# Chlumsky/msdfgen

Hardware: AMD Instinct MI355X
Metric: MSDF glyphs/sec (64x64, fp32) (higher is better)
Workload: dtype f64

## Files before the change

msdfgen_amd/csrc/msdf_ec_fast.hpp:

```cpp
#pragma once

#include "msdf_ec.hpp"

namespace msdfhip {

enum { EC_DEFER = 0x80 };

enum { EC_V_ERROR = 1,
       EC_V_CHECK = 2,
       EC_V_COND = 4,
       EC_V_HELD = 8 };
enum { EC_ORDER_EAGER = 0, EC_ORDER_LAZY = 1, EC_ORDER_LAZY_HELD = 2 };

MSDF_HD bool ecHasBasePass(const EcParams &p) { return p.distanceCheck == EC_DO_NOT_CHECK || (p.distanceCheck == EC_CHECK_AT_EDGE && p.mode != EC_MODE_EDGE_ONLY); }
MSDF_HD bool ecHasShapePass(const EcParams &p) { return p.distanceCheck == EC_ALWAYS_CHECK || p.distanceCheck == EC_CHECK_AT_EDGE; }
MSDF_HD bool ecLazyProtect(const EcParams &p) { return p.mode == EC_MODE_EDGE_PRIORITY && p.distanceCheck == EC_CHECK_AT_EDGE; }

struct FastCtx {
    double span;
    bool p1;
    bool pShape;
    bool basePass, shapePass;
    int order;
};

MSDF_HD int rangeTest2(const FastCtx &c, double at, double bt, double xt, float am, float bm, float xm) {
    const bool inversion = (am > .5f && bm > .5f && xm <= .5f) || (am < .5f && bm < .5f && xm >= .5f);
    const bool outside = medianf(am, bm, xm) != xm;
    const bool candBase = c.basePass && (inversion || (!c.p1 && outside));
    const bool candShape = c.shapePass && (inversion || (!c.pShape && outside));
    const bool candCond = c.order != EC_ORDER_EAGER && !inversion && outside;
    if (!(candBase || candShape || candCond))
        return 0;
    const double axSpan = (xt-at)*c.span, bxSpan = (bt-xt)*c.span;
    const int f = (xm >= am-axSpan && xm <= am+axSpan && xm >= bm-bxSpan && xm <= bm+bxSpan) ? 1 : 3;
    return (candBase ? f : 0)|(candShape ? f<<2 : 0)|(candCond && f == 3 ? 16 : 0);
}

MSDF_HD int judge(int flags) {
    const int cond = (flags&16) ? EC_V_COND : 0;
    if (flags&2)
        return EC_V_ERROR|cond;
    const int fs = (flags>>2)&3;
    if (fs&1)
        return ((fs&2) ? EC_V_ERROR : EC_V_CHECK)|cond;
    return cond;
}

MSDF_HD bool quadraticMayHaveRootInRange(double a, double b, double c) {
    if (a == 0 || fabs(b) > 1e12*fabs(a))
        return true;
    const double lo = .005, hi = .995;
    const double mag = fabs(a)+fabs(b)+fabs(c);
    const double eps = 1e-9*mag;
    const double flo = (a*lo+b)*lo+c, fhi = (a*hi+b)*hi+c;
    if (!(flo > eps && fhi > eps) && !(flo < -eps && fhi < -eps))
        return true;
    const double s = flo > 0 ? 1. : -1.;
    const double as = a*s, bs = b*s, cs = c*s;
    if (as <= 0)
        return false;
    if (!(-bs > 2*as*lo*(1-1e-9) && -bs < 2*as*hi*(1+1e-9)))
        return false;
    return !(4*as*cs-bs*bs > 1e-9*mag*mag);
}

MSDF_HD bool bernsteinMayHaveRoot(float dA, float dBC, float dD) {
    const float m = fmaxf(fmaxf(fabsf(dA), fabsf(dBC)), fabsf(dD));
    const float eps = 1e-5f*m;
    const float h = .5f*dBC;
    return !((dA > eps && h > eps && dD > eps) || (dA < -eps && h < -eps && dD < -eps));
}

MSDF_HD bool edgeBetweenTexelsChannelFast(const float *a, const float *b, int channel) {
    const double n = a[channel]-.5;
    const double d = a[channel]-b[channel];
    if (!((n > 0 && d > 0 && n < d) || (n < 0 && d < 0 && n > d)))
        return false;
    const double t = n/d;
    if (t > 0 && t < 1) {
        float c[3] = { mixf(a[0], b[0], t), mixf(a[1], b[1], t), mixf(a[2], b[2], t) };
        return medianf(c[0], c[1], c[2]) == c[channel];
    }
    return false;
}

MSDF_HD int edgeBetweenTexelsFast(const float *a, const float *b) {
    return 1*(int) edgeBetweenTexelsChannelFast(a, b, 0)+2*(int) edgeBetweenTexelsChannelFast(a, b, 1)+4*(int) edgeBetweenTexelsChannelFast(a, b, 2);
}

template <class Sink>
MSDF_HD int diagonalPairFast(const FastCtx &cx, float am, float dm, const float *a, const float *l, const float *q,
                             float dA, float dBC, float dD, float l0, float q0, float l1, float q1, Sink &sink) {
    const double qa = dD-dBC+dA, qb = dBC-dA-dA, qc = dA;
    if (!quadraticMayHaveRootInRange(qa, qb, qc))
        return 0;
    double t[2];
    const int solutions = solveQuadratic(t, qa, qb, qc);
    int verdict = 0;
    for (int i = 0; i < solutions; ++i) {
        if (t[i] > MSDF_ARTIFACT_T_EPSILON && t[i] < 1-MSDF_ARTIFACT_T_EPSILON) {
            const float xm = interpolatedMedianQuad(a, l, q, t[i]);
            int rangeFlags = rangeTest2(cx, 0, 1, t[i], am, dm, xm);
            const double tEx0 = -.5*l0/q0, tEx1 = -.5*l1/q1;
            if (tEx0 > 0 && tEx0 < 1) {
                double tEnd0 = 0, tEnd1 = 1;
                float em0 = am, em1 = dm;
                const float ex = interpolatedMedianQuad(a, l, q, tEx0);
                if (tEx0 > t[i])
                    tEnd1 = tEx0, em1 = ex;
                else
                    tEnd0 = tEx0, em0 = ex;
                rangeFlags |= rangeTest2(cx, tEnd0, tEnd1, t[i], em0, em1, xm);
            }
            if (tEx1 > 0 && tEx1 < 1) {
                double tEnd0 = 0, tEnd1 = 1;
                float em0 = am, em1 = dm;
                const float ex = interpolatedMedianQuad(a, l, q, tEx1);
                if (tEx1 > t[i])
                    tEnd1 = tEx1, em1 = ex;
                else
                    tEnd0 = tEx1, em0 = ex;
                rangeFlags |= rangeTest2(cx, tEnd0, tEnd1, t[i], em0, em1, xm);
            }
            const int v = judge(rangeFlags);
            verdict |= v;
            if (v&EC_V_CHECK) {
                const bool held = (verdict&EC_V_COND) != 0;
                if (held)
                    verdict |= EC_V_HELD;
                if (held == (cx.order == EC_ORDER_LAZY_HELD))
                    sink(t[i]);
            }
            if (verdict&EC_V_ERROR)
                return verdict;
        }
    }
    return verdict;
}

struct Neighbourhood {
    float v[3][3][3];
    float dev[3][3];
    unsigned valid;
};

MSDF_HD float ecTexelDeviation(const float *t) { return fabsf(medianf(t[0], t[1], t[2])-.5f); }

MSDF_HD void loadNeighbourhood(Neighbourhood &nb, const SdfView &sdf, int x, int yn) {
    nb.valid = 0;
    MSDF_UNROLL
    for (int dy = -1; dy <= 1; ++dy) {
        MSDF_UNROLL
        for (int dx = -1; dx <= 1; ++dx) {
            const int nx = x+dx, ny = yn+dy;
            const bool in = nx >= 0 && ny >= 0 && nx < sdf.w && ny < sdf.h;
            const float *t = sdf.native(in ? nx : x, in ? ny : yn);
            nb.v[dy+1][dx+1][0] = t[0], nb.v[dy+1][dx+1][1] = t[1], nb.v[dy+1][dx+1][2] = t[2];
            nb.dev[dy+1][dx+1] = ecTexelDeviation(t);
            if (in)
                nb.valid |= 1u<<((dy+1)*3+(dx+1));
        }
    }
}

template <class Emit>
MSDF_HD void texelProtectPairs(const Neighbourhood &nb, const EcParams &p, Emit &emit) {
    const float sdev = nb.dev[1][1];
    MSDF_UNROLL
    for (int dy = -1; dy <= 1; ++dy) {
        MSDF_UNROLL
        for (int dx = -1; dx <= 1; ++dx) {
            if (!dx && !dy)
                continue;
            if (!(nb.valid&(1u<<((dy+1)*3+(dx+1)))))
                continue;
            const float radius = dy == 0 ? p.radiusH : dx == 0 ? p.radiusV : p.radiusD;
            const float odev = nb.dev[dy+1][dx+1];
            const bool selfIsA = dy > 0 || (dy == 0 && dx > 0);
            const float sum = selfIsA ? sdev+odev : odev+sdev;
            if (sum < radius)
                emit((dy+1)*3+(dx+1));
        }
    }
}

MSDF_HD bool evaluateProtectPair(const float *self, const float *other, int m) {
    const int dy = m/3-1, dx = m%3-1;
    const bool selfIsA = dy > 0 || (dy == 0 && dx > 0);
    const int mask = selfIsA ? edgeBetweenTexelsFast(self, other) : edgeBetweenTexelsFast(other, self);
    return extremeChannelInMask(self, medianf(self[0], self[1], self[2]), mask);
}

MSDF_HD bool protectedByEdgesNb(const Neighbourhood &nb, const EcParams &p) {
    struct Items {
        unsigned char m[8];
        int n;
        MSDF_HD void operator()(int mm) { m[n++] = (unsigned char) mm; }
    } items;
    items.n = 0;
    texelProtectPairs(nb, p, items);
    for (int i = 0; i < items.n; ++i)
        if (evaluateProtectPair(nb.v[1][1], nb.v[items.m[i]/3][items.m[i]%3], items.m[i]))
            return true;
    return false;
}

MSDF_HD int ecNeighbourDx(int k) { return k < 4 ? (k == 0 ? -1 : k == 2 ? 1 : 0) : ((k&1) ? 1 : -1); }
MSDF_HD int ecNeighbourDy(int k) { return k < 4 ? (k == 1 ? -1 : k == 3 ? 1 : 0) : ((k&2) ? 1 : -1); }

template <class Emit>
MSDF_HD void texelCandidatePairs(const Neighbourhood &nb, Emit &emit) {
    const float *c = nb.v[1][1];
    const float cdev = nb.dev[1][1];
    MSDF_UNROLL
    for (int k = 0; k < 4; ++k) {
        const int dx = k == 0 ? -1 : k == 2 ? 1 : 0, dy = k == 1 ? -1 : k == 3 ? 1 : 0;
        if (!(nb.valid&(1u<<((dy+1)*3+(dx+1)))))
            continue;
        const float *b = nb.v[dy+1][dx+1];
        if (!(cdev >= nb.dev[dy+1][dx+1]))
            continue;
        MSDF_UNROLL
        for (int j = 0; j < 3; ++j) {
            const int i0 = j, i1 = j == 2 ? 0 : j+1;
            const float dA = c[i1]-c[i0], dB = b[i1]-b[i0];
            if ((dA > 0 && dB < 0) || (dA < 0 && dB > 0))
                emit(k, j);
        }
    }
    MSDF_UNROLL
    for (int k = 4; k < 8; ++k) {
        const int dx = (k&1) ? 1 : -1, dy = (k&2) ? 1 : -1;
        if (!(nb.valid&(1u<<((dy+1)*3+(dx+1)))))
            continue;
        const float *d = nb.v[dy+1][dx+1];
        if (!(cdev >= nb.dev[dy+1][dx+1]))
            continue;
        const float *b = nb.v[1][dx+1], *cc = nb.v[dy+1][1];
        MSDF_UNROLL
        for (int j = 0; j < 3; ++j) {
            const int i0 = j, i1 = j == 2 ? 0 : j+1;
            const float dA = c[i1]-c[i0], dBC = b[i1]-b[i0]+cc[i1]-cc[i0], dD = d[i1]-d[i0];
            if (dA == 0 && dBC == 0 && dD == 0)
                continue;
            if (bernsteinMayHaveRoot(dA, dBC, dD))
                emit(k, j);
        }
    }
}

MSDF_HD float pick3(const float *v, int i) { return i == 0 ? v[0] : i == 1 ? v[1] : v[2]; }

template <class Sink>
MSDF_HD int evaluatePair(const float *c, const float *n, const float *hb, const float *vc, const EcParams &p, bool p1, int flip, int k, int j, Sink &sink,
                         int order = EC_ORDER_EAGER) {
    FastCtx cx;
    cx.basePass = ecHasBasePass(p);
    cx.shapePass = ecHasShapePass(p);
    cx.order = order;
    cx.p1 = order != EC_ORDER_EAGER || p1;
    cx.pShape = (p.distanceCheck == EC_CHECK_AT_EDGE) ? true : cx.p1;
    const int dx = ecNeighbourDx(k), dy = ecNeighbourDy(k);
    const int i0 = j, i1 = j == 2 ? 0 : j+1;
    const float cm = medianf(c[0], c[1], c[2]), nm = medianf(n[0], n[1], n[2]);
    if (k < 4) {
        if (order == EC_ORDER_LAZY_HELD)
            return 0;
        cx.span = dy == 0 ? p.hSpan : p.vSpan;
        const float dA = pick3(c, i1)-pick3(c, i0), dB = pick3(n, i1)-pick3(n, i0);
        const double t = (double) dA/(dA-dB);
        if (t > MSDF_ARTIFACT_T_EPSILON && t < 1-MSDF_ARTIFACT_T_EPSILON) {
            const float xm = interpolatedMedianLin(c, n, t);
            const int v = judge(rangeTest2(cx, 0, 1, t, cm, nm, xm));
            if (v&EC_V_CHECK)
                sink(t, dx, flip ? -dy : dy);
            return v;
        }
        return 0;
    }
    cx.span = p.dSpan;
    const float *a = c, *b = hb, *cc = vc, *d = n;
    const float abc[3] = { a[0]-b[0]-cc[0], a[1]-b[1]-cc[1], a[2]-b[2]-cc[2] };
    const float l[3] = { -a[0]-abc[0], -a[1]-abc[1], -a[2]-abc[2] };
    const float q[3] = { d[0]+abc[0], d[1]+abc[1], d[2]+abc[2] };
    const float a3[3] = { a[0], a[1], a[2] };
    struct DirSink {
        Sink &sink;
        int dx, dy;
        MSDF_HD void operator()(double t) { sink(t, dx, dy); }
    } dirSink = { sink, dx, flip ? -dy : dy };
    const float dA = pick3(a, i1)-pick3(a, i0), dBC = pick3(b, i1)-pick3(b, i0)+pick3(cc, i1)-pick3(cc, i0), dD = pick3(d, i1)-pick3(d, i0);
    return diagonalPairFast(cx, cm, nm, a3, l, q, dA, dBC, dD, pick3(l, i0), pick3(q, i0), pick3(l, i1), pick3(q, i1), dirSink);
}

template <class Sink>
MSDF_HD int texelFindFast(const Neighbourhood &nb, const EcParams &p, bool p1, int flip, Sink &sink, int order = EC_ORDER_EAGER) {
    struct Items {
        unsigned char k[24], j[24];
        int n;
        MSDF_HD void operator()(int kk, int jj) { k[n] = (unsigned char) kk, j[n] = (unsigned char) jj; ++n; }
    } items;
    items.n = 0;
    texelCandidatePairs(nb, items);
    int verdict = 0;
    for (int i = 0; i < items.n; ++i) {
        const int k = items.k[i], dx = ecNeighbourDx(k), dy = ecNeighbourDy(k);
        verdict |= evaluatePair(nb.v[1][1], nb.v[dy+1][dx+1], nb.v[1][dx+1], nb.v[dy+1][1], p, p1, flip, k, items.j[i], sink, order);
    }
    return verdict;
}

MSDF_HD bool protectedByCornerList(const int *corners, int nCorners, int x, int ys) {
    for (int i = 0; i < nCorners; ++i) {
        const int l = corners[2*i], b = corners[2*i+1];
        if ((x == l || x == l+1) && (ys == b || ys == b+1))
            return true;
    }
    return false;
}

MSDF_HD bool ecNeedsProtection(int verdict) { return ((verdict&EC_V_COND) && !(verdict&EC_V_ERROR)) || (verdict&EC_V_HELD); }

template <class Sink>
MSDF_HD int ecTexelFast(const SdfView &sdf, const EcParams &p, const int *corners, int nCorners, int x, int yn, Sink &sink, bool allowLazy = true) {
    const int ys = sdf.flip ? sdf.h-1-yn : yn;
    Neighbourhood nb;
    loadNeighbourhood(nb, sdf, x, yn);
    int st = 0, verdict;
    if (allowLazy && ecLazyProtect(p)) {
        verdict = texelFindFast(nb, p, true, sdf.flip, sink, EC_ORDER_LAZY);
        if (ecNeedsProtection(verdict)) {
            if (!(protectedByCornerList(corners, nCorners, x, ys) || protectedByEdgesNb(nb, p)))
                verdict |= EC_V_ERROR;
            else if (verdict&EC_V_HELD)
                texelFindFast(nb, p, true, sdf.flip, sink, EC_ORDER_LAZY_HELD);
        }
    } else {
        if (p.mode == EC_MODE_EDGE_PRIORITY) {
            if (protectedByCornerList(corners, nCorners, x, ys) || protectedByEdgesNb(nb, p))
                st |= EC_PROTECTED;
        } else if (p.mode == EC_MODE_EDGE_ONLY)
            st |= EC_PROTECTED;
        verdict = texelFindFast(nb, p, (st&EC_PROTECTED) != 0, sdf.flip, sink);
    }
    if (ecHasBasePass(p) && p.distanceCheck == EC_CHECK_AT_EDGE)
        st |= EC_PROTECTED;
    if (verdict&EC_V_ERROR)
        st |= EC_ERROR;
    else if (verdict&EC_V_CHECK)
        st |= EC_DEFER;
    return st;
}

template <class Query>
MSDF_HD bool ecEvaluateCandidate(const SdfView &sdf, const EcParams &p, int x, int ys, double t, int dx, int dy, const Query &query) {
    const float *msd = sdf.shape(x, ys);
    const V2 tVector = t*mk(dx, dy);
    float oldMSD[3], newMSD[3];
    interpolate3(oldMSD, sdf, mk(x+.5, ys+.5)+tVector);
    const double aWeight = (1-fabs(tVector.x))*(1-fabs(tVector.y));
    const float aPSD = medianf(msd[0], msd[1], msd[2]);
    newMSD[0] = (float) (oldMSD[0]+aWeight*(aPSD-msd[0]));
    newMSD[1] = (float) (oldMSD[1]+aWeight*(aPSD-msd[1]));
    newMSD[2] = (float) (oldMSD[2]+aWeight*(aPSD-msd[2]));
    const float oldPSD = medianf(oldMSD[0], oldMSD[1], oldMSD[2]);
    const float newPSD = medianf(newMSD[0], newMSD[1], newMSD[2]);
    const V2 q = unproject(p.t, mk(x+.5, ys+.5))+mk(tVector.x*p.texelX, tVector.y*p.texelY);
    const float refPSD = mapDistance(p.t, query(q));
    return p.minImproveRatio*fabsf(newPSD-refPSD) < (double) fabsf(oldPSD-refPSD);
}

}
```

msdfgen_amd/csrc/msdf_kernels.hpp:

```cpp
#pragma once

#include <hip/hip_runtime.h>
#include "msdf_device.hpp"
#include "msdf_prep.hpp"
#include "msdf_ec.hpp"
#include "msdf_ec_fast.hpp"
#include "msdf_cull.hpp"
#include "msdf_scanline.hpp"
#include "msdf_shapeprep.hpp"
#include "msdf_frame.hpp"
#include "../../include/msdfgen_hip.h"

namespace msdfhip {

#ifndef MSDF_DISTANCE_WAVES_PER_SIMD
#define MSDF_DISTANCE_WAVES_PER_SIMD 4
#endif
constexpr int TILE = 8;
constexpr int WAVE = 64;
constexpr int REC_DOUBLES = sizeof(EdgeRec)/sizeof(double);

struct BatchView {
    int nGlyphs;
    const int32_t *glyphContourOffsets;
// ... 845 lines not shown
        return;
    }
    PB contour;
    pbInit(contour);
    const int e = edges.end(c);
    for (int base = edges.begin(c); base < e; base += WAVE) {
        Selector<2> mine;
        selInit(mine);
        const int i = base+edges.lane;
        if (i < e) {
            const EdgeRegs r = loadEdgeRegs(rec+i, i);
            selAddEdge(mine, r, i, o);
        }
        PB &m = mine.c[0];
        MSDF_UNROLL
        for (int off = 1; off < WAVE; off <<= 1) {
            PB other;
            other.td = __shfl_down(m.td, off), other.tdot = __shfl_down(m.tdot, off), other.perp = __shfl_down(m.perp, off);
            other.neg = __shfl_down(m.neg, off), other.pos = __shfl_down(m.pos, off);
            if (edges.lane+off < WAVE)
                pbMerge(m, other);
        }
        PB all;
        all.td = __shfl(m.td, 0), all.tdot = __shfl(m.tdot, 0), all.perp = __shfl(m.perp, 0), all.neg = __shfl(m.neg, 0), all.pos = __shfl(m.pos, 0);
        pbMerge(contour, all);
    }
    pbMerge(sel.c[0], contour);
    if (cacheable) {
        edges.merged[c] = contour;
        edges.cached |= 1ull<<c;
        waveSync();
    }
}

template <bool OVERLAP, class Wind = const int8_t *>
struct PsdfQueryCooperative {
    const EdgeRec *rec;
    const int32_t *coff;
    Wind windings;
    int C, lane;
    double *res;
    PBSlot *slots, *merged;
    int cacheCap = 0;
    __device__ double operator()(V2 q) const {
        double out[1];
        EdgesCooperative edges;
        edges.coff = coff, edges.lane = lane, edges.slots = slots, edges.merged = merged, edges.nE = coff[C]-coff[0], edges.C = C;
        edges.cached = 0, edges.cacheCap = slots ? 0 : cacheCap;
#if defined(MSDF_PROFILE_QUERY)
        for (int i = 0; i < 16; ++i)
            edges.prof[i] = 0;
        const unsigned long long qq0 = qNow();
#endif
        if (slots)
            waveSync();
        if (OVERLAP)
            shapeDistanceOverlap<2>(rec, edges, windings, C, q, res, 1, out);
        else
            shapeDistanceSimple<2>(rec, edges, C, q, out);
#if defined(MSDF_PROFILE_QUERY)
        if (lane == 0) {
            atomicAdd(&gQueryDetail[0], 1ull), atomicAdd(&gQueryDetail[1], qNow()-qq0);
            atomicAdd(&gQueryDetail[2], edges.prof[0]), atomicAdd(&gQueryDetail[3], edges.prof[1]), atomicAdd(&gQueryDetail[4], edges.prof[8]);
            atomicAdd(&gQueryDetail[5], edges.prof[9]), atomicAdd(&gQueryDetail[6], edges.prof[10]), atomicAdd(&gQueryDetail[7], edges.prof[11]);
            atomicAdd(&gQueryDetail[8], (unsigned long long) C), atomicAdd(&gQueryDetail[9], (unsigned long long) (slots ? 1 : 0));
        }
#endif
        return out[0];
    }
};

struct EcCandidate {
    unsigned texel;
    int dir;
    double t;
};
static_assert(sizeof(EcCandidate) == 16, "EcCandidate layout");

MSDF_HD size_t ecHeaderRecords(int nGlyphs) { return ((size_t) (nGlyphs+1)*sizeof(unsigned)+sizeof(EcCandidate)-1)/sizeof(EcCandidate); }
MSDF_HD unsigned ecSegment(size_t texelsPerGlyph) { return (unsigned) (texelsPerGlyph/8 > 64 ? (texelsPerGlyph/8+63)/64*64 : 64); }

struct CandidateSink {
    unsigned *header;
    EcCandidate *segment;
    unsigned seg, texel;
    int g;
    __device__ void operator()(double t, int dx, int dy) {
        const unsigned slot = atomicAdd(&header[1+g], 1u);
        if (slot < seg) {
            EcCandidate c;
            c.texel = texel, c.dir = (dx+1)|((dy+1)<<2), c.t = t;
            segment[slot] = c;
        } else
            header[0] = 1u;
    }
};

MSDF_HD size_t stencilIndex(size_t texel, int yn, int width, int height, int stencilYDown) {
    return stencilYDown ? texel+(size_t) (height-1-2*yn)*width : texel;
}

struct EcGlyphParams {
    double hSpan, vSpan, dSpan, texelX, texelY;
    float radiusH, radiusV, radiusD;
    int cornerBegin, nCorners;
    int pad;
};
static_assert(sizeof(EcGlyphParams) == 64, "EcGlyphParams layout");

__device__ __forceinline__ void ecParamsBody(EcGlyphParams *out, const BatchView &batch, const MsdfHipGlyph *glyphs, const MsdfHipConfig &cfg, unsigned *candidateHeader,
                                             int *corners, int *sizes, const int g, const int lane) {
    if (candidateHeader && lane == 0) {
        candidateHeader[1+g] = 0;
        if (g == 0)
            candidateHeader[0] = 0;
    }
    EcParams p;
    p.t = loadXform(glyphs[g]);
    p.minDeviationRatio = cfg.min_deviation_ratio;
    p.minImproveRatio = cfg.min_improve_ratio;
    ecDerive(p);
    const int c0 = batch.glyphContourOffsets[g], C = batch.glyphContourOffsets[g+1]-c0;
    const int e0 = batch.contourOffsets[c0], nE = batch.contourOffsets[c0+C]-e0;
    int nCorners = 0;
    if (cfg.ec_mode == EC_MODE_EDGE_PRIORITY && corners) {
        const EdgeRec *rec = batch.recs+e0;
        for (int base = 0; base < nE; base += WAVE) {
            const int e = base+lane;
            const bool corner = e < nE && (rec[e].flags&REC_CORNER);
            const unsigned long long mask = __ballot(corner);
            if (corner) {
                const V2 pp = project(p.t, ld(rec[e].p0));
                const int slot = e0+nCorners+__popcll(mask&((1ull<<lane)-1ull));
                corners[2*slot] = (int) floor(pp.x-.5);
                corners[2*slot+1] = (int) floor(pp.y-.5);
            }
            nCorners += __popcll(mask);
        }
    }
    if (lane == 0) {
        EcGlyphParams o;
        o.hSpan = p.hSpan, o.vSpan = p.vSpan, o.dSpan = p.dSpan, o.texelX = p.texelX, o.texelY = p.texelY;
        o.radiusH = p.radiusH, o.radiusV = p.radiusV, o.radiusD = p.radiusD, o.cornerBegin = e0, o.nCorners = nCorners, o.pad = 0;
        out[g] = o;
        if (sizes)
            sizes[2*g] = nE, sizes[2*g+1] = C;
    }
}
__global__ void __launch_bounds__(WAVE)
k_ec_params(EcGlyphParams *out, BatchView batch, const MsdfHipGlyph *glyphs, MsdfHipConfig cfg, unsigned *candidateHeader, int *corners, int *sizes) {
    ecParamsBody(out, batch, glyphs, cfg, candidateHeader, corners, sizes, (int) blockIdx.x, (int) threadIdx.x);
}

#ifndef MSDF_EC_FAST_WAVES_PER_SIMD
#define MSDF_EC_FAST_WAVES_PER_SIMD 7
#endif
enum { EC_HALO = TILE+2, EC_QUEUE_CAP = WAVE*24, EC_PROTECT_QUEUE_CAP = WAVE*8 };
__host__ __device__ inline size_t ecFastLdsBytes(int maxEdges, int n) {
    return (size_t) EC_HALO*EC_HALO*n*sizeof(float)+(WAVE+4)*sizeof(int)
           +(EC_QUEUE_CAP+EC_PROTECT_QUEUE_CAP)*sizeof(unsigned short);
}

__device__ __forceinline__ bool ecTileCornerTexel(const int *list, int nCorners, int tx, int ty, int height, int flip, int lane) {
    const int lxT = lane&(TILE-1), lyT = lane>>3;
    const int xT = tx*TILE+lxT, ysT = flip ? height-1-(ty*TILE+lyT) : ty*TILE+lyT;
    const int x0 = tx*TILE, x1 = tx*TILE+TILE-1;
    const int ya = flip ? height-1-(ty*TILE+TILE-1) : ty*TILE, yb = flip ? height-1-ty*TILE : ty*TILE+TILE-1;
    bool cornerTexel = false;
    for (int base = 0; base < nCorners; base += WAVE) {
        const int k = base+lane;
        int l = 0, b = 0;
        bool near = false;
        if (k < nCorners) {
            l = list[2*k], b = list[2*k+1];
            near = l+1 >= x0 && l <= x1 && b+1 >= ya && b <= yb;
        }
        for (unsigned long long mask = __ballot(near); mask; mask &= mask-1) {
            const int src = __ffsll((long long) mask)-1;
            const int cl = __builtin_amdgcn_readlane(l, src), cb = __builtin_amdgcn_readlane(b, src);
            cornerTexel = cornerTexel || ((xT == cl || xT == cl+1) && (ysT == cb || ysT == cb+1));
        }
    }
    return cornerTexel;
}

template <int N>
__device__ __forceinline__ void ecRunProtectQueue(const float *halo, const unsigned short *protectQueue, int nProtect, int *verdictLds, int lane) {
    for (int base = 0; base < nProtect; base += WAVE) {
        const int it = base+lane;
        if (it >= nProtect)
            continue;
        const unsigned item = protectQueue[it];
        const int s = item&63, m = item>>6;
        const int sx = s&(TILE-1), sy = s>>3;
        const float *self = halo+((sy+1)*EC_HALO+sx+1)*N, *other = halo+((sy+m/3)*EC_HALO+sx+m%3)*N;
        if (evaluateProtectPair(self, other, m))
            atomicOr(&verdictLds[s], 0x100);
    }
}

struct EcPushProtect {
    unsigned short *queue;
    int *count;
    int lane;
    __device__ void operator()(int m) { queue[atomicAdd(count, 1)] = (unsigned short) (lane|m<<6); }
};

template <int N, int ORDER = -1>
__device__ __forceinline__ void ecFastBody(const BatchView &batch, const MsdfHipGlyph *glyphs, int width, int height, int tilesX, int tilesPerGlyph,
          const float *src, float *out, uint8_t *stencilOut, const MsdfHipConfig &cfg, const EcGlyphParams *glyphParams, EcCandidate *cands, unsigned seg,
          int maxEdges, const int *corners, const unsigned blockId, int *smemFast, const int sinkSlots = 0, const int sinkSlot = 0) {
    const GlyphWork wk = decodeItem(blockId, batch.nGlyphs, tilesPerGlyph);
    if (!wk.valid)
        return;
    float *halo = reinterpret_cast<float *>(smemFast);
    int *verdictLds = reinterpret_cast<int *>(halo+EC_HALO*EC_HALO*N);
    int *itemCount = verdictLds+WAVE;
    unsigned short *queue = reinterpret_cast<unsigned short *>(itemCount+4);
    unsigned short *protectQueue = queue+EC_QUEUE_CAP;
    float *devLds = reinterpret_cast<float *>(queue+EC_QUEUE_CAP)-EC_HALO*EC_HALO;
    static_assert((EC_QUEUE_CAP*sizeof(unsigned short))%sizeof(float) == 0 && EC_QUEUE_CAP*sizeof(unsigned short) >= EC_HALO*EC_HALO*sizeof(float), "devLds overlays the queue's tail");
    const int lane = threadIdx.x;
    const MsdfHipGlyph gd = glyphs[wk.g];
    EcParams p;
    p.t = loadXform(gd);
    p.minDeviationRatio = cfg.min_deviation_ratio;
    p.minImproveRatio = cfg.min_improve_ratio;
    p.mode = cfg.ec_mode, p.distanceCheck = cfg.ec_distance_check, p.overlap = cfg.overlap_support, p.stageLimit = 0;
    const EcGlyphParams gp = glyphParams[wk.g];
    p.hSpan = gp.hSpan, p.vSpan = gp.vSpan, p.dSpan = gp.dSpan, p.texelX = gp.texelX, p.texelY = gp.texelY;
    p.radiusH = gp.radiusH, p.radiusV = gp.radiusV, p.radiusD = gp.radiusD;
    const int tx = wk.tile%tilesX, ty = wk.tile/tilesX;

    const bool lazy = ORDER < 0 ? ecLazyProtect(p) : ORDER != 0;
    bool cornerTexel = false;
    if (p.mode == EC_MODE_EDGE_PRIORITY && !lazy)
        cornerTexel = ecTileCornerTexel(corners+2*(size_t) gp.cornerBegin, gp.nCorners, tx, ty, height, gd.flip, lane);

    const float *field = src+(size_t) wk.g*height*width*N;
    for (int idx = lane; idx < EC_HALO*EC_HALO; idx += WAVE) {
        const int hx = tx*TILE+idx%EC_HALO-1, hy = ty*TILE+idx/EC_HALO-1;
        if (hx >= 0 && hy >= 0 && hx < width && hy < height) {
            const float *t = field+((size_t) hy*width+hx)*N;
            float tv[N];
            for (int ch = 0; ch < N; ++ch)
                tv[ch] = t[ch], halo[idx*N+ch] = tv[ch];
            devLds[idx] = ecTexelDeviation(tv);
        }
    }
    if (lane < 2)
        itemCount[lane] = 0;
    waveSync();

    const int lx = lane&(TILE-1), ly = lane>>3;
    const int x = tx*TILE+lx, yn = ty*TILE+ly;
    const bool inside = x < width && yn < height;
    int st = 0;
    const bool classify = inside;
    Neighbourhood nb;
    nb.valid = 0;
    if (classify) {
        MSDF_UNROLL
        for (int dy = -1; dy <= 1; ++dy) {
            MSDF_UNROLL
            for (int dx = -1; dx <= 1; ++dx) {
                const int nx = x+dx, ny = yn+dy;
                const bool in = nx >= 0 && ny >= 0 && nx < width && ny < height;
                const float *t = halo+((ly+1+(in ? dy : 0))*EC_HALO+lx+1+(in ? dx : 0))*N;
                nb.v[dy+1][dx+1][0] = t[0], nb.v[dy+1][dx+1][1] = t[1], nb.v[dy+1][dx+1][2] = t[2];
                nb.dev[dy+1][dx+1] = devLds[(ly+1+(in ? dy : 0))*EC_HALO+lx+1+(in ? dx : 0)];
                if (in)
                    nb.valid |= 1u<<((dy+1)*3+(dx+1));
            }
        }
    }
    waveSync();
    if (classify) {
        if (p.mode == EC_MODE_EDGE_PRIORITY && !lazy) {
            if (cornerTexel)
                st |= EC_PROTECTED;
            if (!(st&EC_PROTECTED)) {
                EcPushProtect pushProtect = { protectQueue, itemCount+1, lane };
                texelProtectPairs(nb, p, pushProtect);
            }
        } else if (p.mode == EC_MODE_EDGE_ONLY)
            st |= EC_PROTECTED;
        struct Push {
            unsigned short *queue;
            int *count;
            int lane;
            __device__ void operator()(int k, int j) { queue[atomicAdd(count, 1)] = (unsigned short) (lane|k<<6|j<<9); }
        } push = { queue, itemCount, lane };
        texelCandidatePairs(nb, push);
    }
    verdictLds[lane] = (st&EC_PROTECTED) ? 0x100 : 0;
    waveSync();

    if (!lazy) {
        ecRunProtectQueue<N>(halo, protectQueue, itemCount[1], verdictLds, lane);
        waveSync();
    }

    const int nItems = itemCount[0];
    const auto runItems = [&](const int order) {
        for (int base = 0; base < nItems; base += WAVE) {
            const int it = base+lane;
            if (it >= nItems)
                continue;
            const unsigned item = queue[it];
            const int s = item&63, k = (item>>6)&7, jp = item>>9;
            const int word = verdictLds[s];
            if (order == EC_ORDER_LAZY_HELD && (word&(0x100|EC_V_HELD)) != (0x100|EC_V_HELD))
                continue;
            const int sx = s&(TILE-1), sy = s>>3;
            const int dx = ecNeighbourDx(k), dy = ecNeighbourDy(k);
            const float *c = halo+((sy+1)*EC_HALO+sx+1)*N, *n = halo+((sy+1+dy)*EC_HALO+sx+1+dx)*N;
            const float *hb = halo+((sy+1)*EC_HALO+sx+1+dx)*N, *vc = halo+((sy+1+dy)*EC_HALO+sx+1)*N;
            CandidateSink sink;
            sink.header = reinterpret_cast<unsigned *>(cands);
            sink.segment = sinkSlots > 0 ? cands+ecHeaderRecords(sinkSlots)+(size_t) sinkSlot*seg : cands+ecHeaderRecords(batch.nGlyphs)+(size_t) wk.g*seg;
            sink.seg = seg, sink.g = sinkSlots > 0 ? sinkSlot : wk.g;
            sink.texel = (unsigned) (((size_t) wk.g*height+ty*TILE+sy)*width+tx*TILE+sx);
            const int v = evaluatePair(c, n, hb, vc, p, (word&0x100) != 0, gd.flip, k, jp, sink, order);
            if (v && order != EC_ORDER_LAZY_HELD)
                atomicOr(&verdictLds[s], v);
        }
    };
    runItems(lazy ? EC_ORDER_LAZY : EC_ORDER_EAGER);
    waveSync();

    const bool need = lazy && inside && ecNeedsProtection(verdictLds[lane]);
    if (__ballot(need)) {
        __asm__ volatile("" ::: "memory");
        const EcGlyphParams gl = glyphParams[wk.g];
        EcParams pr = p;
        pr.radiusH = gl.radiusH, pr.radiusV = gl.radiusV, pr.radiusD = gl.radiusD;
        cornerTexel = ecTileCornerTexel(corners+2*(size_t) gl.cornerBegin, gl.nCorners, tx, ty, height, gd.flip, lane);
        if (need) {
            if (cornerTexel)
                verdictLds[lane] |= 0x100;
            else {
                Neighbourhood nd;
                nd.valid = 0;
                MSDF_UNROLL
                for (int dy = -1; dy <= 1; ++dy) {
                    MSDF_UNROLL
                    for (int dx = -1; dx <= 1; ++dx) {
                        const int nx = x+dx, ny = yn+dy;
                        const bool in = nx >= 0 && ny >= 0 && nx < width && ny < height;
                        nd.dev[dy+1][dx+1] = ecTexelDeviation(halo+((ly+1+(in ? dy : 0))*EC_HALO+lx+1+(in ? dx : 0))*N);
                        if (in)
                            nd.valid |= 1u<<((dy+1)*3+(dx+1));
                    }
                }
                EcPushProtect pushProtect = { protectQueue, itemCount+1, lane };
                texelProtectPairs(nd, pr, pushProtect);
            }
        }
        waveSync();
        ecRunProtectQueue<N>(halo, protectQueue, itemCount[1], verdictLds, lane);
        waveSync();
        bool revisit = false;
        if (need) {
            const int word = verdictLds[lane];
            if (!(word&0x100))
                verdictLds[lane] = word|EC_V_ERROR;
            revisit = (word&0x100) && (word&EC_V_HELD);
        }
        if (__ballot(revisit)) {
            waveSync();
            runItems(EC_ORDER_LAZY_HELD);
        }
    }

    if (!inside)
        return;
    const int verdict = verdictLds[lane];
    if ((verdict&0x100) || (ecHasBasePass(p) && p.distanceCheck == EC_CHECK_AT_EDGE))
        st |= EC_PROTECTED;
    if (verdict&EC_V_ERROR)
        st |= EC_ERROR;
    const size_t texel = ((size_t) wk.g*height+yn)*width+x;
    const float *in = halo+((ly+1)*EC_HALO+lx+1)*N;
    float v[N];
    for (int i = 0; i < N; ++i)
        v[i] = in[i];
    if (st&EC_ERROR) {
        const float m = medianf(v[0], v[1], v[2]);
        v[0] = m, v[1] = m, v[2] = m;
    }
    float *px = out+gd.out_offset+(ptrdiff_t) gd.row_stride*yn+(ptrdiff_t) N*x;
    for (int i = 0; i < N; ++i)
        px[i] = v[i];
    if (stencilOut)
        stencilOut[stencilIndex(texel, yn, width, height, cfg.stencil_y_down)] = (uint8_t) st;
}
template <int N, bool LAZY>
__global__ void __launch_bounds__(WAVE, MSDF_EC_FAST_WAVES_PER_SIMD)
k_ec_fast(BatchView batch, const MsdfHipGlyph *glyphs, int width, int height, int tilesX, int tilesPerGlyph,
          const float *src, float *out, uint8_t *stencilOut, MsdfHipConfig cfg, const EcGlyphParams *glyphParams, EcCandidate *cands, unsigned seg,
          int maxEdges, const int *corners) {
    extern __shared__ int smemFast[];
    ecFastBody<N, LAZY ? 1 : 0>(batch, glyphs, width, height, tilesX, tilesPerGlyph, src, out, stencilOut, cfg, glyphParams, cands, seg, maxEdges, corners, blockIdx.x, smemFast);
}

struct EcQueryPolicy { int lpcMaxContours, lpcEdgeCost, lpcMaxEdges, lpcMinCount, wideMaxEdges; float wideLoad, wideMeanCount; int gridSteps; };
MSDF_HD int ecQueryGridSlices(unsigned count, int nE, int C, EcQueryPolicy q) {
    if (q.gridSteps <= 0 || C > q.lpcMaxContours || count == 0)
        return 0;
    int J = 1;
    while (J < (int) count && J < WAVE)
        J <<= 1;
    int S = WAVE/J, need = 1;
    while (need*q.gridSteps < nE && need < WAVE)
        need <<= 1;
    if (need > S)
        S = need;
    return S >= 2 && S <= WAVE/2 ? S : 0;
}
MSDF_HD bool ecQueryLanePerCandidate(unsigned count, int nE, int C, EcQueryPolicy q) {
    if (C > q.lpcMaxContours)
        return false;
    if ((nE > q.lpcMaxEdges && (int) count < q.lpcMinCount))
        return false;
    const long long coop = (long long) count*(340ll*((nE+WAVE-1)/WAVE)+10ll*nE+1000ll);
    const long long lpc = (long long) ((count+WAVE-1)/WAVE)*((long long) q.lpcEdgeCost*nE+1000ll);
    return lpc < coop;
}
MSDF_HD int ecQueryItems(unsigned count, unsigned seg, int nE, int C, EcQueryPolicy lpcMaxContours) {
    if (count > seg)
        return 0;
    const int S = ecQueryGridSlices(count, nE, C, lpcMaxContours);
    if (S)
        return (int) ((count+WAVE/S-1)/(WAVE/S));
    return ecQueryLanePerCandidate(count, nE, C, lpcMaxContours) ? (int) ((count+WAVE-1)/WAVE) : (int) count;
}
MSDF_HD bool ecQueryListedFirst(unsigned count, int nE, int C, EcQueryPolicy q) {
    return ecQueryGridSlices(count, nE, C, q) != 0 || ecQueryLanePerCandidate(count, nE, C, q) || (q.gridSteps > 0 && nE > WAVE);
}

MSDF_HD size_t ecQueuesAt(int nGlyphs) { return 2*((size_t) nGlyphs+1)+2+2*(size_t) nGlyphs; }
MSDF_HD size_t ecOffsetInts(int nGlyphs) { return ecQueuesAt(nGlyphs)+8*16; }
MSDF_HD size_t ecSizesAt(int nGlyphs) { return 2*((size_t) nGlyphs+1)+2; }

__global__ void __launch_bounds__(1024)
k_ec_scan(int nGlyphs, const unsigned *__restrict__ header, unsigned seg, int *__restrict__ offsets, EcQueryPolicy lpcMaxContours, const int *__restrict__ order) {
    __shared__ int waveTotals[2][16];
    __shared__ float waveLoad[16], waveCount[16];
    enum { PER = 8 };
    const int t = threadIdx.x, lane = t&(WAVE-1), wave = t/WAVE;
    const int *sizes = offsets+ecSizesAt(nGlyphs);
    float mine = 0, mineCount = 0;
    for (int base = 0; base < nGlyphs; base += 1024*PER) {
        unsigned count[PER];
        int nE[PER];
        MSDF_UNROLL
        for (int k = 0; k < PER; ++k) {
            const int p = base+t*PER+k;
            const int g = p < nGlyphs ? (order ? order[p] : p) : -1;
            count[k] = g >= 0 ? header[1+g] : 0u, nE[k] = g >= 0 ? sizes[2*g] : 0;
        }
        MSDF_UNROLL
        for (int k = 0; k < PER; ++k)
            if (count[k] <= seg)
                mine += (float) count[k]*(340.f*((nE[k]+WAVE-1)/WAVE)+10.f*nE[k]+1000.f), mineCount += (float) count[k];
    }
    for (int off = WAVE/2; off > 0; off >>= 1)
        mine += __shfl_down(mine, off), mineCount += __shfl_down(mineCount, off);
    if (lane == 0)
        waveLoad[wave] = mine, waveCount[wave] = mineCount;
    __syncthreads();
    float total = 0, totalCount = 0;
    for (int w = 0; w < 16; ++w)
        total += waveLoad[w], totalCount += waveCount[w];
    const bool dense = lpcMaxContours.wideMeanCount > 0 && totalCount >= lpcMaxContours.wideMeanCount*(float) nGlyphs;
    if ((total > lpcMaxContours.wideLoad || dense) && lpcMaxContours.wideMaxEdges > lpcMaxContours.lpcMaxEdges)
        lpcMaxContours.lpcMaxEdges = lpcMaxContours.wideMaxEdges;
    const bool gridOff = total > lpcMaxContours.wideLoad || dense || lpcMaxContours.gridSteps <= 0;
    if (gridOff)
        lpcMaxContours.gridSteps = 0;
    int *coop = offsets+nGlyphs+1;
    int carry[2] = { 0, 0 };
    for (int base = 0; base < nGlyphs; base += 1024*PER) {
        int items[PER];
        bool chunky[PER];
        int sum[2] = { 0, 0 };
        MSDF_UNROLL
        for (int k = 0; k < PER; ++k) {
            const int p = base+t*PER+k;
            const int g = p < nGlyphs ? (order ? order[p] : p) : -1;
            const unsigned count = g >= 0 ? header[1+g] : 0u;
            const int nE = g >= 0 ? sizes[2*g] : 0, C = g >= 0 ? sizes[2*g+1] : 0;
            chunky[k] = g >= 0 && ecQueryListedFirst(count, nE, C, lpcMaxContours);
            items[k] = g >= 0 ? ecQueryItems(count, seg, nE, C, lpcMaxContours) : 0;
            sum[chunky[k] ? 0 : 1] += items[k];
        }
        int incl[2] = { sum[0], sum[1] };
        for (int off = 1; off < WAVE; off <<= 1) {
            const int n0 = __shfl_up(incl[0], off), n1 = __shfl_up(incl[1], off);
            if (lane >= off)
                incl[0] += n0, incl[1] += n1;
        }
        if (lane == WAVE-1)
            waveTotals[0][wave] = incl[0], waveTotals[1][wave] = incl[1];
        __syncthreads();
        int before[2] = { 0, 0 }, all[2] = { 0, 0 };
        for (int w = 0; w < 16; ++w) {
            const int v0 = waveTotals[0][w], v1 = waveTotals[1][w];
            if (w < wave)
                before[0] += v0, before[1] += v1;
            all[0] += v0, all[1] += v1;
        }
        int at[2] = { carry[0]+before[0]+incl[0]-sum[0], carry[1]+before[1]+incl[1]-sum[1] };
        MSDF_UNROLL
        for (int k = 0; k < PER; ++k) {
            const int p = base+t*PER+k;
            if (p < nGlyphs) {
                offsets[p] = at[0], coop[p] = at[1];
                at[chunky[k] ? 0 : 1] += items[k];
            }
        }
        carry[0] += all[0], carry[1] += all[1];
        __syncthreads();
    }
    if (t == 1023) {
        offsets[nGlyphs] = carry[0];
        coop[nGlyphs] = carry[1];
        coop[nGlyphs+1] = 0;
        for (int q = 0; q < 8; ++q)
            offsets[ecQueuesAt(nGlyphs)+16*q] = 0;
        coop[nGlyphs+2] = lpcMaxContours.lpcMaxEdges|(gridOff ? 1<<30 : 0);
    }
}

#ifndef MSDF_EC_QUERY_WAVES_PER_SIMD
#define MSDF_EC_QUERY_WAVES_PER_SIMD 3
#endif
#if defined(MSDF_PROFILE_QUERY)
__device__ unsigned long long gQueryProfile[24];
#if MSDF_PROFILE_QUERY >= 2
#define MSDF_QSTAMP(x) asm volatile("s_waitcnt vmcnt(0) lgkmcnt(0)" ::: "memory"); const unsigned long long x = __builtin_readcyclecounter()
#else
#define MSDF_QSTAMP(x) const unsigned long long x = __builtin_readcyclecounter()
#endif
#endif
template <int N, bool OVERLAP>
__global__ void __launch_bounds__(WAVE, MSDF_EC_QUERY_WAVES_PER_SIMD)
k_ec_query(int nGlyphs, const int32_t *__restrict__ glyphContourOffsets, const int32_t *__restrict__ contourOffsets, const EdgeRec *__restrict__ recs,
           const int8_t *__restrict__ windings, const MsdfHipGlyph *__restrict__ glyphs, int width, int height, const float *__restrict__ src, float *__restrict__ out,
           uint8_t *__restrict__ stencilOut, MsdfHipConfig cfg, const EcGlyphParams *__restrict__ glyphParams, const EcCandidate *__restrict__ cands, unsigned seg,
           const int *__restrict__ offsets, int *__restrict__ counter, int itemsPerTicket, int slotCap, int slotOffset, EcQueryPolicy lpcMaxContours,
           unsigned *__restrict__ overflowOut, const int *__restrict__ order, int queryFlags) {
    if (overflowOut && blockIdx.x == 0 && threadIdx.x == 0)
        *overflowOut = reinterpret_cast<const unsigned *>(cands)[0];
    BatchView batch;
    batch.nGlyphs = nGlyphs, batch.glyphContourOffsets = glyphContourOffsets, batch.contourOffsets = contourOffsets, batch.recs = recs, batch.windings = windings;
    extern __shared__ double smemLds[];
    PBSlot *slotBuf = reinterpret_cast<PBSlot *>(smemLds+slotOffset);
    const unsigned *header = reinterpret_cast<const unsigned *>(cands);
    const size_t texelsPerGlyph = (size_t) width*height;
    const int chunks = offsets[batch.nGlyphs], coopItems = offsets[2*batch.nGlyphs+1];
    const int tickets = chunks+(coopItems+itemsPerTicket-1)/itemsPerTicket;
    lpcMaxContours.lpcMaxEdges = offsets[2*batch.nGlyphs+3]&((1<<30)-1);
    if (offsets[2*batch.nGlyphs+3]&(1<<30))
        lpcMaxContours.gridSteps = 0;
#if defined(MSDF_PROFILE_QUERY)
    MSDF_QSTAMP(qStart);
    unsigned long long qAcc[8] = { 0, 0, 0, 0, 0, 0, 0, 0 }, qItems[4] = { 0, 0, 0, 0 }, qLongest = 0, qLastWork = 0, qLongestWho = 0;
#endif
    const int dealt = (queryFlags&1) ? (int) gridDim.x : 0;
    for (int round = 0;; ++round) {
#if defined(MSDF_PROFILE_QUERY)
        MSDF_QSTAMP(q0);
#endif
        int ticket = 0;
        if (dealt && (queryFlags&4) && round > 0) {
            const int q = (int) blockIdx.x&7;
            if (threadIdx.x == 0)
                ticket = atomicAdd(counter+(ecQueuesAt(batch.nGlyphs)-(2*(size_t) batch.nGlyphs+2))+16*q, 1);
            ticket = dealt+__builtin_amdgcn_readfirstlane(ticket)*8+q;
            if (ticket >= tickets)
                break;
        } else if (dealt) {
            if ((long long) round*dealt >= tickets)
                break;
            ticket = (round&1) ? (round+1)*dealt-1-(int) blockIdx.x : round*dealt+(int) blockIdx.x;
            if (ticket >= tickets)
                continue;
        } else {
            if (threadIdx.x == 0)
                ticket = atomicAdd(counter, 1);
            ticket = __builtin_amdgcn_readfirstlane(ticket);
            if (ticket >= tickets)
                break;
        }
#if defined(MSDF_PROFILE_QUERY)
        MSDF_QSTAMP(q1);
        qAcc[0] += q1-q0;
#endif
        const int *part = ticket < chunks ? offsets : offsets+batch.nGlyphs+1;
        const int first = ticket < chunks ? ticket : (ticket-chunks)*itemsPerTicket;
        const int last = ticket < chunks ? first+1 : (first+itemsPerTicket < coopItems ? first+itemsPerTicket : coopItems);
        int lo = 0, hi = batch.nGlyphs-1;
        while (lo < hi) {
            const int mid = (lo+hi)>>1;
            if (part[mid+1] > first)
                hi = mid;
            else
                lo = mid+1;
        }
        int pos = lo;
        MSDF_NOUNROLL
        for (int i = first; i < last; ++i) {
#if defined(MSDF_PROFILE_QUERY)
        MSDF_QSTAMP(q2a);
#endif
        while (part[pos+1] <= i)
            ++pos;
        const int item = i-part[pos];
        const int g = order ? order[pos] : pos;
#if defined(MSDF_PROFILE_QUERY)
        MSDF_QSTAMP(q2);
        qAcc[1] += q2-(i == first ? q1 : q2a);
#endif
        const unsigned count = header[1+g];
        const EcCandidate *segment = cands+ecHeaderRecords(batch.nGlyphs)+(size_t) g*seg;
        const int c0 = batch.glyphContourOffsets[g], C = batch.glyphContourOffsets[g+1]-c0;
        const int32_t *coff = batch.contourOffsets+c0;
        const MsdfHipGlyph gd = glyphs[g];
        EcParams p;
        p.t = loadXform(gd);
        p.minDeviationRatio = cfg.min_deviation_ratio;
        p.minImproveRatio = cfg.min_improve_ratio;
        p.mode = cfg.ec_mode, p.distanceCheck = cfg.ec_distance_check, p.overlap = OVERLAP, p.stageLimit = 0;
        const EcGlyphParams gp = glyphParams[g];
        p.hSpan = gp.hSpan, p.vSpan = gp.vSpan, p.dSpan = gp.dSpan, p.texelX = gp.texelX, p.texelY = gp.texelY;
        p.radiusH = gp.radiusH, p.radiusV = gp.radiusV, p.radiusD = gp.radiusD;
        SdfView sdf;
        sdf.px = src+(size_t) g*texelsPerGlyph*N;
        sdf.w = width, sdf.h = height, sdf.N = N, sdf.flip = gd.flip;
        const int nE = coff[C]-coff[0];
        WindingMasks wind;
        wind.mem = batch.windings+c0;
        wind.pos = wind.neg = 0;
        if (OVERLAP) {
            const int w = (int) threadIdx.x < C ? (int) wind.mem[threadIdx.x] : 0;
            wind.pos = __ballot(w > 0), wind.neg = __ballot(w < 0);
        }
#if defined(MSDF_PROFILE_QUERY)
        MSDF_QSTAMP(q3);
        qAcc[2] += q3-q2;
        unsigned long long q4 = q3;
        const bool qChunk = ecQueryListedFirst(count, nE, C, lpcMaxContours);
#endif
        const int gridS = ecQueryGridSlices(count, nE, C, lpcMaxContours);
        if (gridS) {
            PsdfQueryGrid<OVERLAP, WindingMasks> query;
            query.rec = batch.recs+coff[0], query.coff = coff, query.windings = wind, query.C = C, query.res = smemLds+threadIdx.x;
            query.S = gridS, query.slice = (int) threadIdx.x&(gridS-1);
            const unsigned k = (unsigned) item*(unsigned) (WAVE/gridS)+threadIdx.x/(unsigned) gridS;
            if (k < count) {
                const EcCandidate cand = segment[k];
                const size_t texel = cand.texel;
                const int rem = (int) (texel-(size_t) g*texelsPerGlyph);
                const int yn = rem/width, x = rem%width;
                const int ys = gd.flip ? height-1-yn : yn;
                const bool artifact = ecEvaluateCandidate(sdf, p, x, ys, cand.t, (cand.dir&3)-1, ((cand.dir>>2)&3)-1, query);
                if (artifact && query.slice == 0) {
                    const float *in = sdf.native(x, yn);
                    const float m = medianf(in[0], in[1], in[2]);
                    float *px = out+gd.out_offset+(ptrdiff_t) gd.row_stride*yn+(ptrdiff_t) N*x;
                    px[0] = m, px[1] = m, px[2] = m;
                    if (stencilOut)
                        stencilOut[stencilIndex(texel, yn, width, height, cfg.stencil_y_down)] |= (uint8_t) EC_ERROR;
// ... 598 lines not shown
```

Before: 1.824 million.

## Split diagonal pair evaluation into filter and compacted heavy stages with lazy settle test

```diff
diff --git a/msdfgen_amd/csrc/msdf_ec_fast.hpp b/msdfgen_amd/csrc/msdf_ec_fast.hpp
--- a/msdfgen_amd/csrc/msdf_ec_fast.hpp
+++ b/msdfgen_amd/csrc/msdf_ec_fast.hpp
@@ -11,6 +11,8 @@
        EC_V_COND = 4,
        EC_V_HELD = 8 };
 enum { EC_ORDER_EAGER = 0, EC_ORDER_LAZY = 1, EC_ORDER_LAZY_HELD = 2 };
+enum { EC_STAGE_ALL = 0, EC_STAGE_FILTER = 1, EC_STAGE_HEAVY = 2 };
+enum { EC_V_HEAVY = 0x40 };
 
 MSDF_HD bool ecHasBasePass(const EcParams &p) { return p.distanceCheck == EC_DO_NOT_CHECK || (p.distanceCheck == EC_CHECK_AT_EDGE && p.mode != EC_MODE_EDGE_ONLY); }
 MSDF_HD bool ecHasShapePass(const EcParams &p) { return p.distanceCheck == EC_ALWAYS_CHECK || p.distanceCheck == EC_CHECK_AT_EDGE; }
@@ -89,12 +91,45 @@
     return 1*(int) edgeBetweenTexelsChannelFast(a, b, 0)+2*(int) edgeBetweenTexelsChannelFast(a, b, 1)+4*(int) edgeBetweenTexelsChannelFast(a, b, 2);
 }
 
+MSDF_HD float pick3(const float *v, int i) { return i == 0 ? v[0] : i == 1 ? v[1] : v[2]; }
+
+MSDF_HD bool diagonalSettledLazy(const float *a, const float *b, const float *cc, const float *d, const float *l, const float *q, float am, float dm,
+                                 int i0, int i1, float qa, double dSpan) {
+    const bool finite = fabsf(q[0])+fabsf(q[1])+fabsf(q[2]) <= 3.4e38f;
+    const float l0 = pick3(l, i0), q0 = pick3(q, i0), l1 = pick3(l, i1), q1 = pick3(q, i1);
+    const float al0 = fabsf(l0), aq0 = fabsf(q0), al1 = fabsf(l1), aq1 = fabsf(q1);
+    const bool ex0 = (al0 > 0)&((l0 < 0) != (q0 < 0))&(al0 < 2*aq0);
+    const bool ex1 = (al1 > 0)&((l1 < 0) != (q1 < 0))&(al1 < 2*aq1);
+    float m = fmaxf(fmaxf(fabsf(a[0]), fabsf(a[1])), fabsf(a[2]));
+    m = fmaxf(m, fmaxf(fmaxf(fabsf(b[0]), fabsf(b[1])), fabsf(b[2])));
+    m = fmaxf(m, fmaxf(fmaxf(fabsf(cc[0]), fabsf(cc[1])), fabsf(cc[2])));
+    m = fmaxf(m, fmaxf(fmaxf(fabsf(d[0]), fabsf(d[1])), fabsf(d[2])));
+    const float m1 = m+1.f;
+    const bool residual = (qa == 0)|(fabsf(qa)*m1 >= 1e-8f*m*m);
+    const float e = 4e-5f*m1;
+    const float lim = (float) dSpan*(1-1e-6f)-100*e;
+    const float a0 = pick3(a, i0), a1 = pick3(a, i1), d0 = pick3(d, i0), d1 = pick3(d, i1);
+    const float s0 = al0+aq0, s1 = al1+aq1;
+    const bool endA = ((am == a0)&(s0 <= lim))|((am == a1)&(s1 <= lim));
+    const bool endD = ((dm == d0)&(s0+aq0 <= lim))|((dm == d1)&(s1+aq1 <= lim));
+    const bool above = (am > .5f)&(dm > .5f), below = (am < .5f)&(dm < .5f);
+    const bool clearAbove = fmaxf(fminf(a0, d0), fminf(a1, d1))-e > .5f;
+    const bool clearBelow = fminf(fmaxf(a0, d0), fmaxf(a1, d1))+e < .5f;
+    const bool noInversion = (!above|clearAbove)&(!below|clearBelow);
+    return finite&!ex0&!ex1&residual&endA&endD&noInversion;
+}
+
+MSDF_HD bool diagonalSettledLazyTexels(const float *a, const float *b, const float *cc, const float *d, int i0, int i1, double dSpan) {
+    const float abc[3] = { a[0]-b[0]-cc[0], a[1]-b[1]-cc[1], a[2]-b[2]-cc[2] };
+    const float l[3] = { -a[0]-abc[0], -a[1]-abc[1], -a[2]-abc[2] };
+    const float q[3] = { d[0]+abc[0], d[1]+abc[1], d[2]+abc[2] };
+    const float dA = pick3(a, i1)-pick3(a, i0), dBC = pick3(b, i1)-pick3(b, i0)+pick3(cc, i1)-pick3(cc, i0), dD = pick3(d, i1)-pick3(d, i0);
+    return diagonalSettledLazy(a, b, cc, d, l, q, medianf(a[0], a[1], a[2]), medianf(d[0], d[1], d[2]), i0, i1, dD-dBC+dA, dSpan);
+}
+
 template <class Sink>
-MSDF_HD int diagonalPairFast(const FastCtx &cx, float am, float dm, const float *a, const float *l, const float *q,
-                             float dA, float dBC, float dD, float l0, float q0, float l1, float q1, Sink &sink) {
-    const double qa = dD-dBC+dA, qb = dBC-dA-dA, qc = dA;
-    if (!quadraticMayHaveRootInRange(qa, qb, qc))
-        return 0;
+MSDF_HD int diagonalPairHeavy(const FastCtx &cx, float am, float dm, const float *a, const float *l, const float *q,
+                              double qa, double qb, double qc, float l0, float q0, float l1, float q1, Sink &sink) {
     double t[2];
     const int solutions = solveQuadratic(t, qa, qb, qc);
     int verdict = 0;
@@ -250,11 +285,9 @@
     }
 }
 
-MSDF_HD float pick3(const float *v, int i) { return i == 0 ? v[0] : i == 1 ? v[1] : v[2]; }
-
 template <class Sink>
 MSDF_HD int evaluatePair(const float *c, const float *n, const float *hb, const float *vc, const EcParams &p, bool p1, int flip, int k, int j, Sink &sink,
-                         int order = EC_ORDER_EAGER) {
+                         int order = EC_ORDER_EAGER, int stage = EC_STAGE_ALL) {
     FastCtx cx;
     cx.basePass = ecHasBasePass(p);
     cx.shapePass = ecHasShapePass(p);
@@ -291,7 +324,17 @@
         MSDF_HD void operator()(double t) { sink(t, dx, dy); }
     } dirSink = { sink, dx, flip ? -dy : dy };
     const float dA = pick3(a, i1)-pick3(a, i0), dBC = pick3(b, i1)-pick3(b, i0)+pick3(cc, i1)-pick3(cc, i0), dD = pick3(d, i1)-pick3(d, i0);
-    return diagonalPairFast(cx, cm, nm, a3, l, q, dA, dBC, dD, pick3(l, i0), pick3(q, i0), pick3(l, i1), pick3(q, i1), dirSink);
+    const float qaf = dD-dBC+dA;
+    const double qa = qaf, qb = dBC-dA-dA, qc = dA;
+    if (stage != EC_STAGE_HEAVY) {
+        if (order != EC_ORDER_EAGER && diagonalSettledLazy(a, b, cc, d, l, q, cm, nm, i0, i1, qaf, p.dSpan))
+            return 0;
+        if (!quadraticMayHaveRootInRange(qa, qb, qc))
+            return 0;
+        if (stage == EC_STAGE_FILTER)
+            return EC_V_HEAVY;
+    }
+    return diagonalPairHeavy(cx, cm, nm, a3, l, q, qa, qb, qc, pick3(l, i0), pick3(q, i0), pick3(l, i1), pick3(q, i1), dirSink);
 }
 
 template <class Sink>
diff --git a/msdfgen_amd/csrc/msdf_kernels.hpp b/msdfgen_amd/csrc/msdf_kernels.hpp
--- a/msdfgen_amd/csrc/msdf_kernels.hpp
+++ b/msdfgen_amd/csrc/msdf_kernels.hpp
@@ -1171,31 +1171,46 @@
     }
 
     const int nItems = itemCount[0];
-    const auto runItems = [&](const int order) {
-        for (int base = 0; base < nItems; base += WAVE) {
-            const int it = base+lane;
-            if (it >= nItems)
-                continue;
-            const unsigned item = queue[it];
-            const int s = item&63, k = (item>>6)&7, jp = item>>9;
-            const int word = verdictLds[s];
-            if (order == EC_ORDER_LAZY_HELD && (word&(0x100|EC_V_HELD)) != (0x100|EC_V_HELD))
-                continue;
-            const int sx = s&(TILE-1), sy = s>>3;
-            const int dx = ecNeighbourDx(k), dy = ecNeighbourDy(k);
-            const float *c = halo+((sy+1)*EC_HALO+sx+1)*N, *n = halo+((sy+1+dy)*EC_HALO+sx+1+dx)*N;
-            const float *hb = halo+((sy+1)*EC_HALO+sx+1+dx)*N, *vc = halo+((sy+1+dy)*EC_HALO+sx+1)*N;
-            CandidateSink sink;
-            sink.header = reinterpret_cast<unsigned *>(cands);
-            sink.segment = sinkSlots > 0 ? cands+ecHeaderRecords(sinkSlots)+(size_t) sinkSlot*seg : cands+ecHeaderRecords(batch.nGlyphs)+(size_t) wk.g*seg;
-            sink.seg = seg, sink.g = sinkSlots > 0 ? sinkSlot : wk.g;
-            sink.texel = (unsigned) (((size_t) wk.g*height+ty*TILE+sy)*width+tx*TILE+sx);
-            const int v = evaluatePair(c, n, hb, vc, p, (word&0x100) != 0, gd.flip, k, jp, sink, order);
-            if (v && order != EC_ORDER_LAZY_HELD)
-                atomicOr(&verdictLds[s], v);
-        }
+    const auto runItem = [&](const unsigned item, const int order, const int stage) {
+        const int s = item&63, k = (item>>6)&7, jp = item>>9;
+        const int word = verdictLds[s];
+        if (order == EC_ORDER_LAZY_HELD && (word&(0x100|EC_V_HELD)) != (0x100|EC_V_HELD))
+            return 0;
+        const int sx = s&(TILE-1), sy = s>>3;
+        const int dx = ecNeighbourDx(k), dy = ecNeighbourDy(k);
+        const float *c = halo+((sy+1)*EC_HALO+sx+1)*N, *n = halo+((sy+1+dy)*EC_HALO+sx+1+dx)*N;
+        const float *hb = halo+((sy+1)*EC_HALO+sx+1+dx)*N, *vc = halo+((sy+1+dy)*EC_HALO+sx+1)*N;
+        CandidateSink sink;
+        sink.header = reinterpret_cast<unsigned *>(cands);
+        sink.segment = sinkSlots > 0 ? cands+ecHeaderRecords(sinkSlots)+(size_t) sinkSlot*seg : cands+ecHeaderRecords(batch.nGlyphs)+(size_t) wk.g*seg;
+        sink.seg = seg, sink.g = sinkSlots > 0 ? sinkSlot : wk.g;
+        sink.texel = (unsigned) (((size_t) wk.g*height+ty*TILE+sy)*width+tx*TILE+sx);
+        const int v = evaluatePair(c, n, hb, vc, p, (word&0x100) != 0, gd.flip, k, jp, sink, order, stage);
+        if ((v&~EC_V_HEAVY) && order != EC_ORDER_LAZY_HELD)
+            atomicOr(&verdictLds[s], v&~EC_V_HEAVY);
+        return v&EC_V_HEAVY;
     };
-    runItems(lazy ? EC_ORDER_LAZY : EC_ORDER_EAGER);
+    int nHeavy = 0;
+    for (int base = 0; base < nItems; base += WAVE) {
+        const int it = base+lane;
+        unsigned item = 0;
+        bool heavy = false;
+        if (it < nItems) {
+            item = queue[it];
+            heavy = runItem(item, lazy ? EC_ORDER_LAZY : EC_ORDER_EAGER, EC_STAGE_FILTER) != 0;
+        }
+        const unsigned long long survivors = __ballot(heavy);
+        if (heavy)
+            queue[nHeavy+(int) __builtin_amdgcn_mbcnt_hi((unsigned) (survivors>>32), __builtin_amdgcn_mbcnt_lo((unsigned) survivors, 0u))] = (unsigned short) item;
+        nHeavy += __popcll(survivors);
+    }
+    waveSync();
+    const auto runHeavy = [&](const int order) {
+        for (int base = 0; base < nHeavy; base += WAVE)
+            if (base+lane < nHeavy)
+                runItem(queue[base+lane], order, EC_STAGE_HEAVY);
+    };
+    runHeavy(lazy ? EC_ORDER_LAZY : EC_ORDER_EAGER);
     waveSync();
 
     const bool need = lazy && inside && ecNeedsProtection(verdictLds[lane]);
@@ -1238,7 +1253,7 @@
         }
         if (__ballot(revisit)) {
             waveSync();
-            runItems(EC_ORDER_LAZY_HELD);
+            runHeavy(EC_ORDER_LAZY_HELD);
         }
     }
 
```

After: 1.837 million (median of 6 runs). No clear change (+0.7%).
